# osudrl/cassie-mujoco-sim

Hardware: AMD Instinct MI355X
Metric: env-steps/sec (whole node) at N envs; max |qpos_err| vs CPU ref (higher is better)
Workload: dtype f64

## Files before the change

cassie-mujoco-sim_amd/cassie_amd/_lib.py:

```python
import ctypes
import os

from . import cstruct

PKG_DIR = os.path.dirname(os.path.dirname(os.path.abspath(__file__)))
REPO_DIR = os.path.dirname(PKG_DIR)
LIB_PATH = os.environ.get("CASSIE_LIB") or os.path.join(PKG_DIR, "lib", "libcassiemujoco.so")
MODEL_DIR = os.path.join(REPO_DIR, "models")

_variant_hdr = LIB_PATH + ".cm_model.h"
with open(_variant_hdr if os.path.exists(_variant_hdr) else os.path.join(PKG_DIR, "csrc", "cm_model.h")) as _f:
    _hdr = _f.read()
MACROS = cstruct.parse_defines(_hdr)
_structs = cstruct.parse_structs(_hdr, MACROS)
CmModel = _structs["cm_model_t"]
CmDriveState = _structs["cm_drive_state_t"]
CmEnvParams = _structs["cm_envparams_t"]
CmEpisodeRules = _structs.get("cm_episode_rules_t")

_lib = None


def lib():
    global _lib
# ... 74 lines not shown
    L.phys_batch_download_drive_state.argtypes = [vp, vp, c.c_int, c.c_int]
    L.phys_batch_uses_applied.argtypes = [vp]
    L.phys_batch_drive_pass.argtypes = [vp, c.c_int, vp]
    L.phys_batch_mark.argtypes = [vp]
    L.phys_batch_debug_poison_lds.argtypes = [vp]
    L.phys_batch_set_balance.argtypes = [vp, c.c_int]
    L.phys_batch_set_fast_rows.argtypes = [vp, c.c_int]
    L.phys_batch_set_waves_per_env.argtypes = [vp, c.c_int]
    L.phys_batch_set_inplace.argtypes = [vp, c.c_int]
    L.phys_batch_debug_inplace_ranges.argtypes = [vp]
    L.phys_batch_debug_form_launches.argtypes = [vp, c.POINTER(c.c_longlong), c.POINTER(c.c_longlong)]
    L.phys_batch_download_cost.argtypes = [vp, vp]
    L.phys_batch_measured_shader_clock.argtypes = [vp, vp]
    L.phys_batch_wide_pass_envs.argtypes = [vp, c.c_int]
    L.phys_batch_set_chunks.argtypes = [vp, c.c_int]
    L.phys_batch_debug_handover_pending.argtypes = [vp]
    L.phys_batch_debug_handover_pending.restype = c.c_int
    if hasattr(L, "phys_batch_kernel_timing"):
        L.phys_batch_enable_kernel_timing.argtypes = [vp, c.c_int]
        L.phys_batch_kernel_timing.argtypes = [vp, c.POINTER(c.c_int), c.POINTER(c.c_double)]
    if hasattr(L, "phys_batch_step_range"):
        L.phys_batch_step_range.argtypes = [vp, c.c_int, c.c_int, c.c_int, vp]
    if hasattr(L, "phys_batch_reset_envs"):
        L.phys_batch_reset_envs.argtypes = [vp, c.c_int, c.c_int, c.c_int, vp, vp, vp]
    if hasattr(L, "phys_batch_end_episodes"):
        L.phys_batch_episodes_enable.argtypes = [vp, c.POINTER(CmEpisodeRules)]
        L.phys_batch_episodes_set_bank.argtypes = [vp, vp, c.c_int, c.c_int]
        L.phys_batch_episode_row_dim.argtypes = [vp]
        L.phys_batch_episode_ptr.restype = vp
        L.phys_batch_episode_ptr.argtypes = [vp, c.c_int]
# ... 24 lines not shown
```

cassie-mujoco-sim_amd/cassie_amd/phys.py:

```python
import ctypes
import os

import numpy as np

from ._lib import CmDriveState, CmEnvParams, CmEpisodeRules, CmModel, MODEL_DIR, lib

(F_QPOS, F_QVEL, F_QACC_WARMSTART, F_TIME, F_CTRL, F_QFRC_APPLIED, F_XFRC_APPLIED, F_QACC, F_SENSORDATA,
 F_ACTUATOR_VELOCITY, F_XPOS, F_XQUAT, F_PD_PTARGET, F_PD_KP, F_PD_KD, F_BODY_CFRC, F_DRIVE_CMD, F_MEAS, F_PD_DTARGET,
 F_PD_TORQUE, F_DERIVED, F_QM, F_HEIGHT_SCAN) = range(23)

MAXV = 40
DRV_COM_POS, DRV_COM_VEL, DRV_ANGMOM, DRV_FOOT_POS, DRV_FOOT_VEL, DRV_FOOT_FORCE, DRV_TOE_FORCE, DRV_HEEL_FORCE, DRV_MASS = 0, 3, 6, 9, 15, 27, 39, 45, 51
DRV_FOOT_JACP, DRV_FOOT_JACR, DRV_DIM = 52, 52 + 6 * MAXV, 52 + 12 * MAXV

DRIVE_OFF, DRIVE_TORQUE, DRIVE_PD, DRIVE_PD_SAFE = 0, 1, 2, 3
SAFETY_MSG_LIMIT, SAFETY_MSG_TORQUE = 1, 2
MEAS_DRIVE_POS, MEAS_DRIVE_VEL, MEAS_DRIVE_TORQUE, MEAS_JOINT_POS, MEAS_JOINT_VEL = 0, 10, 20, 30, 36
MEAS_ORIENTATION, MEAS_ANGVEL, MEAS_LINACC, MEAS_MAG, MEAS_DIM = 42, 46, 49, 52, 56

FLAG_EULERDAMP, FLAG_WARMSTART, FLAG_REFSAFE, FLAG_HFDENSE, FLAG_HFMULTI, FLAG_HFPRISM, FLAG_BOX8 = 1, 2, 4, 8, 16, 32, 64
WARN_CONTACT_FULL, WARN_CONSTRAINT_FULL, WARN_UNSUPPORTED_PAIR, WARN_DIVERGED = 1, 2, 4, 8
WARN_CHUNK_PLACEMENT = 16
WARN_TERRAIN_INDEX = 32
WARN_SCAN_TILTED = 64
# ... 370 lines not shown
        a, c_ = ctypes.c_longlong(0), ctypes.c_longlong(0)
        lib().phys_batch_debug_form_launches(self._h, ctypes.byref(a), ctypes.byref(c_))
        return int(a.value), int(c_.value)

    def inplace_ranges(self):
        return lib().phys_batch_debug_inplace_ranges(self._h)

    def set_waves_per_env(self, waves=2):
        if lib().phys_batch_set_waves_per_env(self._h, int(waves)) != 0:
            raise ValueError("waves per env: 1 or 2")

    def set_chunks(self, chunks=4):
        if lib().phys_batch_set_chunks(self._h, int(chunks)) != 0:
            raise ValueError("chunks per env-launch: 1 .. 7")

    def launch_cost(self):
        out = np.zeros(self.nenv, dtype=np.uint32)
        if lib().phys_batch_download_cost(self._h, out.ctypes.data) != 0:
            raise RuntimeError("cost download failed (balancing is off or the batch is small)")
        return out.astype(np.float64) * 64.0

    def measured_shader_clock(self):
        import ctypes
        hz = ctypes.c_double(0.0)
        if lib().phys_batch_measured_shader_clock(self._h, ctypes.byref(hz)) != 0:
            return None
        return float(hz.value)

    def wide_pass_envs(self, env0=0):
        r = lib().phys_batch_wide_pass_envs(self._h, int(env0))
# ... 43 lines not shown
```

cassie-mujoco-sim_amd/csrc/env_step_rows.inc:

```
        int r_ = lane;
        int rtype = -1, rid = 0, rsub = 0;
        int nefc = 0, nefc_before_contacts = 0;
        double rpos = 0, rmargin = 0, rR = 1.0, rK = 0, rB = 0, rimp = 1.0;
        const bool need_imu = lastsub || io.all_outputs_every_substep || (io.drive_mode && sub + 2 == nsub);
        const bool need_pos = lastsub || io.drive_mode || io.all_outputs_every_substep;
        const bool issens = lane < m->nsensor && need_pos;
        const int ls = issens ? lane : 0;
        SensorConsts sens_c;
        double ycol[NVP];
        double jvel = 0, jws = 0;
        const bool lastcol = !WIDE && lane == NROW - 1;
        for (int pass = 0; pass < (WIDE ? 2 : 1); ++pass) {
        if constexpr (WIDE) {
            if (pass == 1 && nefc <= NROW) break;
            r_ = NROW * pass + lane; rtype = -1; rid = 0; rsub = 0; nefc = 0; jvel = 0; jws = 0;
            rpos = 0; rmargin = 0; rR = 1.0; rK = 0; rB = 0; rimp = 1.0;
        }
        {
            const int neq = m->neq;
            const bool eact = lane < neq && m->eq_active[lane < neq ? lane : 0] != 0;
            const unsigned long long eall = neq >= 64 ? ~0ull : (1ull << neq) - 1;
            if (wv::ballot(eact) == eall && 3 * neq <= capr) {
                if (r_ < 3 * neq) { rtype = CM_CNSTR_EQUALITY; rid = r_ / 3; rsub = r_ - 3 * rid; }
                nefc = 3 * neq;
// ... 206 lines not shown
            if (!WIDE && rtype == CM_CNSTR_EQUALITY && r_ < CM_MAXEQROW) {
                ex->eq_pos[r_] = rpos; ex->eq_id[r_] = rid;
#pragma unroll
                for (int k = 0; k < NVP; ++k) if (k < nv) ex->eq_J[r_][k] = ycol[k];
            }
            if (lane == 0) { int ne = 0; for (int e = 0; e < m->neq; ++e) if (m->eq_active[e] && ne + 3 <= capr) ne += 3; ex->ne = ne; }
            if (lane < ncon) {
                ex->con_geom1[lane] = m->geom_fullid[S.c_g1[lane]]; ex->con_geom2[lane] = m->geom_fullid[S.c_g2[lane]];
                ex->con_body1[lane] = m->geom_bodyid[S.c_g1[lane]]; ex->con_body2[lane] = m->geom_bodyid[S.c_g2[lane]];
                ex->con_dim[lane] = S.c_dim[lane]; ex->con_dist[lane] = S.c_dist[lane];
                for (int i = 0; i < 3; ++i) ex->con_pos[lane][i] = S.c_pos[lane][i];
                for (int i = 0; i < 9; ++i) ex->con_frame[lane][i] = S.c_frame[lane][i];
            }
        }
        int caddr = -1;
        const bool want_cfrc = io.body_cfrc && (sub == nsub - 1 || !io.integrate);
        if (io.ext || want_cfrc) {
            int acc = nefc_before_contacts;
            for (int c = 0; c < ncon; ++c) {
                const int dim = S.c_dim[c];
                if (dim != 1 && dim != 3) continue;
                const int nrow = dim == 1 ? 1 : 2 * (dim - 1);
                if (acc + nrow > capr) continue;
                if (c == lane) caddr = acc;
                acc += nrow;
            }
        }
        wv::sync();
        CK_STAMP(8);
```

cassie-mujoco-sim_amd/csrc/env_step_wave1.inc:

```
    if constexpr (NW == 2) {
        if (wid == 1) {
            for (int sub1 = sub_start;;) {
                const int pb = isbody ? b : 0;
                const double mass = P->body_mass[pb];
                double iner[3], imat[9];
                for (int i = 0; i < 3; ++i) iner[i] = P->body_inertia[pb][i];
                for (int i = 0; i < 9; ++i) imat[i] = m->body_imat[pb][i];
                CK_STAMP(35);
                wv::block_barrier();
                if (wv::opaque(S.cmd[0])) return -1;
                wv::set_priority<(FEAT & FEAT_HFIELD) != 0 ? CK_PRIO_W1_FJ_HFIELD : CK_PRIO_W1_FJ>();
                CK_STAMP(36);
                double ximat[9] = {1, 0, 0, 0, 1, 0, 0, 0, 1};
                if (isbody && b > 0) {
                    double xm[9];
                    for (int i = 0; i < 9; ++i) xm[i] = S.x.s.xmat[b][i];
                    for (int i = 0; i < 3; ++i)
                        for (int c = 0; c < 3; ++c) ximat[3 * i + c] = xm[3 * i] * imat[c] + xm[3 * i + 1] * imat[3 + c] + xm[3 * i + 2] * imat[6 + c];
                }
                double col[NVP], colh[NVP];
                mass_matrix_columns<NVP, TOPO, FEAT, NW>(io, S, m, env, ids, mass, iner, ximat, col, colh);
                wv::publish(&S.cmd[3], sub1 + 1);
                CK_STAMP(38);
                factor_pair_by_height<NVP, TOPO, 0>(m, P, h, S, col, colh, lane);
                constexpr bool park_colh = NVP > 32;
                if constexpr (park_colh) {
                    if (isdof) {
#pragma unroll
                        for (int i = 0; i < NVP; ++i) {
                            if (i >= TOPO::nv) continue;
                            if (i == k_) S.dinvH[k_] = colh[i];
                            else if (i > k_ && LP::col_has(i, k_)) S.LHp[LP::col_idx(i, k_)] = colh[i];
                        }
                    }
                    wv::sync();
                }
                wv::wait_for(&S.cmd[4], sub1 + 1);
                if (wv::opaque(S.cmd[0])) return -1;
                if (io.drive_mode) {
                    if (io.integrate) drive_level_io(io, S, m, env, lane, sub1 == nsub - 1);
                    wv::sync();
                }
                CK_STAMP(4);
                {
                    const int kd = isdof ? k_ : 0;
                    const double kdamp = P->dof_damping[kd], kstiff = PS->dof_stiffness[kd], kref = PS->dof_springref[kd];
                    const double kgear = m->dof_gear[kd], klo = m->dof_ctrl_lo[kd], khi = m->dof_ctrl_hi[kd];
                    const int kq = m->dof_qadr[kd], ka = m->dof_act[kd];
                    wv::wait_for(&S.cmd[1], sub1 + 1);
                    bias_forces_and_qfrc_smooth<NVP, (NVP > 32)>(io, S, m, env, ids, kdamp, kstiff, kref, kgear, klo, khi, kq, ka);
                }
                const bool lastsub1 = sub1 == nsub - 1 || !io.integrate;
                const bool need_imu1 = lastsub1 || io.all_outputs_every_substep || (io.drive_mode && sub1 + 2 == nsub);
                const bool issens1 = lane < m->nsensor && (lastsub1 || io.drive_mode || io.all_outputs_every_substep);
                const int ls1 = issens1 ? lane : 0;
                const SensorConsts sens_c1 = request_sensor_consts(m, ls1);
                const int aslot1 = sensors_before_solve(io, S, m, env, issens1, ls1, sens_c1, need_imu1, lastsub1);
                CK_STAMP(47);
                wv::block_barrier();
                wv::set_priority<CK_PRIO_W1_JP>();
                CK_STAMP(39);
                if constexpr (WIDE) {
                    int it1 = 0, ng1 = 0;
                    const double f1 = wide_solve<NVP, TOPO>(S, m, P, 1, wv::opaque(S.x.turn[0]), sub1, it1, ng1);
                    (&S.c_solimp[0][0])[NROW + lane] = f1;
                }
                if constexpr (park_colh) {
#pragma unroll
// ... 76 lines not shown
                    }
                    if (isdof) S.qacc[k_] = qacc;
                    const double av = pf_agear * S.qvel[pf_adof];
                    wv::sync();
                    CK_STAMP(12);
                    if (io.integrate) {
                        if constexpr (!stage_h_early) stage_factor_h<NVP, TOPO>(S, k_, isdof, nv, lcol, lrowh);
                        euler_step<NVP, TOPO>(S, m, lane, isdof, k_, nv, njnt, h, qacc, lcol, lrowh, dih, pf_kdamp, pf_ejt, pf_eqa, pf_eda);
                    }
                    CK_STAMP(13);
                    wv::block_barrier();
                    wv::set_priority<CK_PRIO_W1_EF>();
                    outputs_after_qacc(io, S, m, env, lane, isdof, k_, nu, qacc, aslot, sb, need_imu, lastsub, av, ncon, nefc, iters, nguarded);
                    CK_STAMP(14);
                }
                if (!io.integrate || ++sub1 >= nsub) return -1;
            }
        }
    }
```

cassie-mujoco-sim_amd/csrc/phys_batch.hip:

```cpp
#include <hip/hip_runtime.h>

#include <cstdio>
#include <cstdlib>
#include <cstring>
#include <string>
#include <utility>
#include <vector>

#include "cassie_phys.h"
#include "device_mem.h"
#include "small_kernels.h"
#include "step_launch.h"

void phys_set_last_error(const char *s);

constexpr int DEFAULT_CHUNKS_WHOLE = 7 , DEFAULT_CHUNKS_RANGE = 2, CHUNK_MIN_ENVS = 2048, CHUNK_MIN_SUBSTEPS = 5;
constexpr int DEFAULT_TRAY_WAVES = 2;

struct phys_batch {
    int nenv = 0, device = 0;
    cm_model_t host_model;
    DevBuf<cm_model_t> d_models;
    DevBuf<cm_envparams_t> d_envparams;
    int model_stride = 0;
    bool generic_kernel = false;
    int dim[PHYS_F_COUNT];
    int stride[PHYS_F_COUNT];
    DevBuf<double> d_field[PHYS_F_COUNT];
    DevBuf<int> d_warn, d_info;
    DevBuf<float> d_hfield;
    size_t hfield_stride = 0, hfield_floats = 0;
// ... 20 lines not shown
    std::vector<OrderSeg> order_segs;
    std::vector<int> order_ident;
    DevBuf<cm_ext_t> d_ext;
    bool timing = false;
    std::vector<std::pair<hipEvent_t, hipEvent_t>> ev_pool;
    size_t ev_used = 0;
    DevBuf<int> d_progress;
    int chunks = DEFAULT_CHUNKS_WHOLE, chunks_range = DEFAULT_CHUNKS_RANGE;
    bool chunks_default = true;
    DevBuf<int> d_chunk_flag;
    int chunk_seq = 0;
    bool chunks_allowed = true;
    std::vector<std::pair<hipStream_t, bool>> probed_streams;
    HostWords chunk_fault;
    bool chunk_fault_reported = false;
    DevBuf<int> d_handover_list, d_handover_count;
    HostWords handover_seen;
    DevBuf<int> d_handover_list2, d_handover_count2;
    HostWords handover_seen2;
    bool fast_rows = true;
    int inplace_mode = 2;
    struct RangeForm { int env0; bool inplace; };
    std::vector<RangeForm> range_forms;
    long long form_launches[2] = {0, 0};
    int waves_per_env = 2;
    int waves_per_env_tray = DEFAULT_TRAY_WAVES;
    DevBuf<double> d_scratch_out;
    bool episodes = false;
    cm_episode_rules_t ep_rules;
    DevBuf<char> d_ep[PHYS_EP_ARRAYS];
// ... 127 lines not shown
    launch_step<40, TopoCassieTray38, ck::FEAT_WAVEPAIRS, FAST_ROWS_TRAY>,
    launch_step<40, TopoCassieTray38, ck::FEAT_WAVEPAIRS, FAST_ROWS_TRAY, 2>,
    nullptr,
    launch_step<40, TopoCassieTray38, ck::FEAT_WAVEPAIRS, MID_ROWS, 1, true>,
    launch_step<40, TopoCassieTray38, ck::FEAT_WAVEPAIRS, MID_ROWS, 2, true>,
    nullptr,
};
static const ck::StepLauncher CASSIE_ALL_FORMS[ck::FORM_COUNT] = {launch_step<32, TopoCassie32, ck::FEAT_ALL>};
static const ck::StepLauncher TRAY_HFIELD_FORMS[ck::FORM_COUNT] = {launch_step<40, TopoCassieTray38, ck::FEAT_ALL>};
static const ck::StepLauncher GENERIC32_FORMS[ck::FORM_COUNT] = {launch_step<32, TopoRuntime, ck::FEAT_ALL>};
static const ck::StepLauncher GENERIC40_FORMS[ck::FORM_COUNT] = {launch_step<40, TopoRuntime, ck::FEAT_ALL>};

constexpr int SMALL_BATCH_NSUB = 4;
constexpr int SMALL_BATCH = 512;

static void set_chunks(phys_batch *b, ck::PhysIO &io, int n, int nsub, hipStream_t s) {
    io.nchunk = 1;
    if (!b->chunks_allowed || (n == b->nenv ? b->chunks : b->chunks_range) <= 1 || n < CHUNK_MIN_ENVS || n % 8 != 0 || nsub < 2 * CHUNK_MIN_SUBSTEPS ||
        !stream_may_chunk(b, s))
        return;
    const int range_chunks = b->chunks_default && nsub <= 25 ? 3 : b->chunks_range;
    const int most = nsub / CHUNK_MIN_SUBSTEPS, asked = n == b->nenv ? b->chunks : range_chunks;
    io.nchunk = asked < most ? asked : most;
    if (b->chunk_seq >= (1 << 24)) {
        (void)hipDeviceSynchronize();
        (void)hipMemsetAsync(b->d_chunk_flag, 0, sizeof(int) * (size_t)b->nenv, s);
        (void)hipStreamSynchronize(s);
        b->chunk_seq = 0;
    }
    io.chunk_seq = ++b->chunk_seq;
    io.chunk_flag = b->d_chunk_flag;
    io.chunk_fault = b->chunk_fault.dev();
}

static void range_lists(phys_batch *b, int env0, int n, bool wide, ck::HandoverLists &hl, ck::StepGrids &g) {
    hl.list1 = b->d_handover_list; hl.count1 = b->d_handover_count + 2 * (size_t)env0; hl.seen1 = b->handover_seen.dev() + env0;
    if (wide) { hl.list2 = b->d_handover_list2; hl.count2 = b->d_handover_count2 + 2 * (size_t)env0; hl.seen2 = b->handover_seen2.dev() + env0; }
    const int seen = b->handover_seen.host()[env0], seen2 = wide ? b->handover_seen2.host()[env0] : 0;
// ... 182 lines not shown
        if (f == PHYS_F_DERIVED || f == PHYS_F_QM) continue;
        if (f == PHYS_F_HEIGHT_SCAN) continue;
        ok = ok && b->d_field[f].alloc(n * (d[f] > 0 ? d[f] : 1), true, "field");
    }
    ok = ok && b->d_models.alloc(1, false, "model");
    ok = ok && hip_ok(hipMemcpy(b->d_models, model, sizeof(cm_model_t), hipMemcpyHostToDevice), "hipMemcpy(model)");
    ok = ok && b->d_warn.alloc(n, true, "warn") && b->d_info.alloc(4 * n, true, "info");
    if (nenv >= 2048) {
        b->order_ident.resize(n);
        for (int e = 0; e < nenv; ++e) b->order_ident[(size_t)e] = e;
        ok = ok && b->d_order.alloc(n, false, "order");
        ok = ok && hip_ok(hipMemcpy(b->d_order, b->order_ident.data(), sizeof(int) * n, hipMemcpyHostToDevice), "hipMemcpy(order)");
        ok = ok && b->d_cost.alloc(n, true, "cost") && b->d_cost_wall.alloc(n, true, "cost, wall clock");
    }
    ok = ok && b->d_progress.alloc(n, true, "progress") && b->d_chunk_flag.alloc(n, true, "chunk words");
    if (const char *ck = getenv("CASSIE_CHUNKS")) { b->chunks = b->chunks_range = atoi(ck) > 1 ? (atoi(ck) < 7 ? atoi(ck) : 7) : 1; b->chunks_default = false; }
    ok = ok && b->chunk_fault.alloc(1, "chunk fault word");
    ok = ok && b->d_handover_list.alloc(n, false, "hand-over list") && b->d_handover_count.alloc(2 * n, true, "hand-over counts");
    ok = ok && b->handover_seen.alloc(n, "hand-over seen");
    ok = ok && b->d_handover_list2.alloc(n, false, "second hand-over list") && b->d_handover_count2.alloc(2 * n, true, "second hand-over counts");
    ok = ok && b->handover_seen2.alloc(n, "second hand-over seen");
    ok = ok && hip_ok(hipStreamCreateWithFlags(&b->stream, hipStreamNonBlocking), "hipStreamCreate");
    ok = ok && hip_ok(hipEventCreate(&b->ev0), "hipEventCreate") && hip_ok(hipEventCreate(&b->ev1), "hipEventCreate");
    ok = ok && hip_ok(hipEventCreateWithFlags(&b->ev_mark, hipEventDisableTiming), "hipEventCreate");
    if (ok) {
        std::vector<double> q0((size_t)nenv * model->nq);
        for (int e = 0; e < nenv; ++e) memcpy(&q0[(size_t)e * model->nq], model->qpos0, sizeof(double) * model->nq);
        ok = hip_ok(hipMemcpy(b->d_field[PHYS_F_QPOS], q0.data(), q0.size() * sizeof(double), hipMemcpyHostToDevice),
                    "hipMemcpy(qpos0)");
    }
// ... 663 lines not shown
}

int phys_batch_set_inplace(phys_batch_t *b, int mode) {
    if (!b || mode < 0 || mode > 2) return -1;
    b->inplace_mode = mode;
    return 0;
}

int phys_batch_set_chunks(phys_batch_t *b, int chunks) {
    if (!b || chunks < 1 || chunks > 7) return -1;
    b->chunks = b->chunks_range = chunks;
    b->chunks_default = false;
    return 0;
}

int phys_batch_set_waves_per_env(phys_batch_t *b, int waves) {
    if (!b || (waves != 1 && waves != 2)) return -1;
    b->waves_per_env = waves;
    b->waves_per_env_tray = waves;
    return 0;
}

int phys_batch_download_cost(phys_batch_t *b, unsigned *host) {
    if (!b || !host || !b->d_cost) return -1;
    (void)hipSetDevice(b->device);
    return quiesce(b) && hip_ok(hipMemcpy(host, b->d_cost, sizeof(unsigned) * (size_t)b->nenv, hipMemcpyDeviceToHost), "cost download") ? 0 : -1;
}

int phys_batch_measured_shader_clock(phys_batch_t *b, double *hz) {
    if (!b || !hz || !b->d_cost || !b->d_cost_wall) return -1;
// ... 90 lines not shown
```

cassie-mujoco-sim_amd/csrc/physics_kernel.h:

```cpp
#ifndef CASSIE_PHYSICS_KERNEL_H
#define CASSIE_PHYSICS_KERNEL_H

#include <wave.h>

#include "cm_model.h"
#include "topo_static.h"

#include "pk_types.h"
#include "pk_math.h"
#include "pk_safety.h"
#include "pk_collision.h"
#include "pk_factor_solve.h"
#include "pk_stages.h"
#include "pk_wide_solve.h"

namespace ck {


constexpr int ENV_STEP_WENT_DOWN = 1 << 20;

template <int NVP, class TOPO, int FEAT, int MAXR, int NW>
WV_DEVICE int env_step(const PhysIO &io, EnvShared<NVP, LPack<TOPO, NVP>::count, MAXR> &S, int env, int sub_start, int nsub) {
    typedef LPack<TOPO, NVP> LP;
    static_assert(NW == 1 || NW == 2, "one or two wavefronts per env");
    static_assert(NW == 1 || TOPO::is_static, "the two-wave form exists for the compile-time topologies");
    const int wid = NW == 2 ? wv::wave_id() : 0;
    if constexpr (NW == 2) { if (wid == 0) wv::set_priority<CK_PRIO_W0>(); }
    constexpr int prio_kin = (FEAT & FEAT_HFIELD) != 0 ? CK_PRIO_W0 : CK_PRIO_W0_KIN;

    static_assert(LP::covers() && LP::distinct(), "packed factor rows must hold every ancestor pair, each in its own slot");
    typedef EnvShared<NVP, LPack<TOPO, NVP>::count, MAXR> SH_T;
    constexpr int MAXC = SH_T::MAXC;
    constexpr bool WIDE = SH_T::WIDE;
    static_assert(!WIDE || (NW == 2 && MAXR == WIDE_ROWS), "the 127-row instantiation spreads its solve over the two wavefronts of an env");
    const ModelPtr m_launch = (ModelPtr)(io.models + (size_t)env * io.model_stride);
    ModelPtr m = m_launch;
    const ParamPtr P = io.envparams ? (ParamPtr)(io.envparams + (size_t)env) : (ParamPtr)&m_launch->params;
// ... 51 lines not shown
    const LaneIds ids = {nbody, nv, broot, bend, kjnt, kbody, kjt, kda, kroot, kbend, kdesc};
    wv::sync();

#include "env_step_wave1.inc"

    const float *env_hfield = nullptr;
    if constexpr ((FEAT & FEAT_HFIELD) != 0) {
        bool clamped;
        env_hfield = terrain_grid(io.hfield, io.hfield_stride, io.hfield_index, io.hfield_nterrain, env, &clamped);
        if (clamped && lane == 0 && wid == 0) wv::atomic_or(io.warn + env, WARN_TERRAIN_INDEX);
    }

    bool bailed = false, bailed_down = false;
    int sub = sub_start;
    for (; sub < nsub; ++sub) {
        const bool lastsub = sub == nsub - 1 || !io.integrate;
        const bool need_quat = lastsub || io.ext != nullptr || io.all_outputs_every_substep || (io.drive_mode && sub + 2 == nsub);
        {
            bool badv = false;
            if (lane < nq) { double v = S.qpos[lane]; badv |= !(v == v) || fabs(v) > 1e10; }
            if (lane < nv) { double v = S.qvel[lane]; badv |= !(v == v) || fabs(v) > 1e10; }
            if (wv::ballot(badv) != 0ull) {
                warn |= WARN_DIVERGED;
                if constexpr (NW == 2) { if (lane == 0) S.cmd[0] = 1; wv::block_barrier(); }
                break;
            }
        }
        if (io.drive_mode) {
        } else if (io.pd_ptarget) {
            if (lane < nu) {
                const size_t o = (size_t)env * io.su + lane;
                const double ratio = m->act_gear[lane], tmax = m->act_ctrlrange[lane][1];
// ... 311 lines not shown
        } else bias_forces_and_qfrc_smooth<NVP>(io, S, m, env, ids, kdamp, kstiff, kref, kgear, klo, khi, kq, ka);
        const int pf_eq = lane < 3 * m->neq ? lane / 3 : 0;
        int pf_eb1 = m->eq_body1[pf_eq], pf_eb2 = m->eq_body2[pf_eq], pf_er1 = m->eq_root[pf_eq][0], pf_er2 = m->eq_root[pf_eq][1];

#include "env_step_rows.inc"

#include "env_step_solve.inc"

    if (io.progress && lane == 0 && (!io.resume || bailed)) {
        io.progress[env] = bailed ? sub : nsub;
        if (bailed && !bailed_down && io.handover_out_list) io.handover_out_list[io.env0 + wv::atomic_add(io.handover_out_count, 1)] = env;
    }
    if (io.integrate && io.drive_mode) {
        drive_state_store(io, S, env, lane);
        if (lane < nu) io.ctrl[(size_t)env * io.su + lane] = S.ctrl[lane];
        if (bailed) {
            if (lane < m->nsensordata) io.sensordata[(size_t)env * io.ssd + lane] = S.sens[lane];
            if (lane < nu) io.actuator_velocity[(size_t)env * io.su + lane] = S.actvel[lane];
            if (lane < CM_NUM_DRIVES) {
                double *meas = io.meas + (size_t)env * CM_MEAS_DIM;
                meas[CM_MEAS_DRIVE_POS + lane] = S.drv_pos[lane]; meas[CM_MEAS_DRIVE_VEL + lane] = S.drv_vel[lane];
            }
        }
    }
    if (io.integrate) {
        if (lane < nq) io.qpos[(size_t)env * io.sq + lane] = S.qpos[lane];
        if (lane < nv) {
            io.qvel[(size_t)env * io.sqv + lane] = S.qvel[lane];
            io.qacc_warmstart[(size_t)env * io.sv + lane] = S.qacc_ws[lane];
        }
        if (lane == 0) io.time[env] = time;
    }
    {
        int w = 0;
        for (int bit = 1; bit <= 8; bit <<= 1)
            if (wv::ballot((warn & bit) != 0) != 0ull) w |= bit;
        if (lane == 0 && w) io.warn[env] |= w;
    }
    return (warn & WARN_DIVERGED) ? -2 : (bailed ? (bailed_down ? sub | ENV_STEP_WENT_DOWN : sub) : nsub);
}

template <int NVP, class TOPO, int FEAT = FEAT_ALL, int MAXR = MID_ROWS, int NW = 1, bool WALK = false, int WPS = NW, int INROWS = 0>
WV_GLOBAL void __launch_bounds__(WV_WAVE * NW) WV_OCC WV_WAVES_PER_SIMD(WPS) cassie_step_kernel(PhysIO io) {
    WV_SHARED EnvShared<NVP, LPack<TOPO, NVP>::count, MAXR> S;
    const int slot = wv::env_id();
    if constexpr (WALK) {
        wv::test_launch_hook(&S, sizeof S);
        const int count = wv::opaque(wv::shfl_i(wv::lane() == 0 ? wv::atomic_add(io.handover_count, 0) : 0, 0));
        for (int idx = slot; idx < count; idx += wv::grid_size()) {
            const int env = io.handover_list[io.env0 + idx];
            const long long t0 = io.cost ? wv::clock() : 0, t0w = io.cost_wall ? wv::wall_clock() : 0;
            env_step<NVP, TOPO, FEAT, MAXR, NW>(io, S, env, io.progress[env], io.nsub);
            if (io.cost && wv::lane() == 0 && (NW == 1 || wv::wave_id() == 0)) {
                io.cost[env] += (unsigned)((wv::clock() - t0) >> 6);
                if (io.cost_wall) io.cost_wall[env] += (unsigned)(wv::wall_clock() - t0w);
            }
            if constexpr (NW == 2) wv::block_barrier();
            else wv::sync();
        }
        if (wv::lane() == 0 && (NW == 1 || wv::wave_id() == 0) && wv::atomic_add(io.handover_count + 1, 1) == wv::grid_size() - 1) {
            io.handover_count[0] = 0; io.handover_count[1] = 0;
            if (io.handover_seen) *io.handover_seen = count;
        }
    } else {
    const int chunk = io.nchunk > 1 ? wv::env_id() / io.nenv : 0;
    const int eslot = slot - chunk * io.nenv;
    if (chunk >= (io.nchunk > 1 ? io.nchunk : 1)) return;
    wv::test_launch_hook(&S, sizeof S);
    const int env = io.order ? io.order[io.env0 + eslot] : io.env0 + eslot;
    int sub_start = io.resume ? io.progress[env] : 0, sub_end = io.nsub;
    if (io.nchunk > 1) {
        const int per = (io.nsub + io.nchunk - 1) / io.nchunk;
        sub_start = chunk * per;
        sub_end = sub_start + per < io.nsub ? sub_start + per : io.nsub;
    }
    if (sub_start >= io.nsub) return;
    if (chunk > 0) {
        if (!wv::wait_global<NW>(io.chunk_flag + env, io.chunk_seq, chunk)) {
            if (wv::lane() == 0) { wv::atomic_or(io.warn + env, WARN_CHUNK_PLACEMENT); if (io.chunk_fault) *io.chunk_fault = 1; }
        }
        if (io.progress[env] != sub_start) {
            if (sub_end < io.nsub) wv::publish_global<NW>(io.chunk_flag + env, io.chunk_seq, chunk + 1);
            return;
        }
    }
    const long long t0 = io.cost ? wv::clock() : 0, t0w = io.cost_wall ? wv::wall_clock() : 0;
    if constexpr (INROWS > 0) {
        static_assert(NW == 2 && INROWS > MAXR && INROWS <= MID_ROWS, "the in-place form: a two-wave fast instantiation with the 63-row code behind it");
        static_assert(sizeof(EnvShared<NVP, LPack<TOPO, NVP>::count, MAXR>) == sizeof(EnvShared<NVP, LPack<TOPO, NVP>::count, INROWS>), "both instantiations use the env's LDS block alike");
        auto &S2 = reinterpret_cast<EnvShared<NVP, LPack<TOPO, NVP>::count, INROWS> &>(S);
        PhysIO io2 = io;
        io2.has_next = io.inplace_has_next; io2.handover_out_list = io.inplace_out_list; io2.handover_out_count = io.inplace_out_count;
        io2.down_rows = io.inplace_stay_rows;
        const bool stay = io.inplace_stay_rows > 0;
        bool did = false;
        for (int s = sub_start;;) {
            int at = env_step<NVP, TOPO, FEAT, MAXR, NW>(io, S, env, s, sub_end);
            if (wv::lane() == 0 && wv::wave_id() == 0) S.cmd[5] = at;
            wv::drain_vmem(); wv::block_barrier();
            at = wv::opaque(S.cmd[5]);
            if (at < 0 || at >= sub_end) break;
            did = true;
            int at2 = env_step<NVP, TOPO, FEAT, INROWS, NW>(io2, S2, env, at, stay ? sub_end : at + 1);
            if (wv::lane() == 0 && wv::wave_id() == 0) S.cmd[5] = at2;
            wv::drain_vmem(); wv::block_barrier();
            at2 = wv::opaque(S.cmd[5]);
            if (at2 < 0) break;
            const bool down = (at2 & ENV_STEP_WENT_DOWN) != 0;
            at2 &= ENV_STEP_WENT_DOWN - 1;
            if (at2 >= sub_end) break;
            if (stay ? !down : at2 != at + 1) break;
            s = at2;
        }
        if (did && io.inplace_count && wv::lane() == 0 && wv::wave_id() == 0) wv::atomic_add(io.inplace_count, 1);
    } else env_step<NVP, TOPO, FEAT, MAXR, NW>(io, S, env, sub_start, sub_end);
    if (sub_end < io.nsub) wv::publish_global<NW>(io.chunk_flag + env, io.chunk_seq, chunk + 1);
    if (io.prof && wv::lane() == 0) io.prof[(size_t)env * NSTAMP + 40 + (NW == 2 ? wv::wave_id() : 0)] = wv::hw_id();
    if (io.prof && wv::lane() == 0 && (NW == 1 || wv::wave_id() == 0)) {
        io.prof[(size_t)env * NSTAMP + 42] = wv::clock(); io.prof[(size_t)env * NSTAMP + 43] = wv::wall_clock();
    }
    if (io.cost && wv::lane() == 0 && (NW == 1 || wv::wave_id() == 0)) {
        const unsigned c = (unsigned)((wv::clock() - t0) >> 6);
        io.cost[env] = io.resume || chunk > 0 ? io.cost[env] + c : c;
        if (io.cost_wall) { const unsigned cw = (unsigned)(wv::wall_clock() - t0w); io.cost_wall[env] = io.resume || chunk > 0 ? io.cost_wall[env] + cw : cw; }
    }
    }
}

}
#endif
// ... 1 lines not shown
```

cassie-mujoco-sim_amd/csrc/pk_stages.h:

```cpp
#ifndef CASSIE_PK_STAGES_H
#define CASSIE_PK_STAGES_H

namespace ck {

WV_DEVICE int drive_sensor_slot(int i) { return i < 5 ? i : i + 3; }
WV_DEVICE int joint_sensor_slot(int j) { return j < 3 ? j + 5 : j + 10; }

#define WV_DRIVE_FN WV_DEVICE
template <class SH>
WV_DEVICE void drive_state_load(const PhysIO &io, SH &S, int env, int lane) {
    const cm_drive_state_t *ds = io.drive_state + env;
    const double *meas = io.meas + (size_t)env * CM_MEAS_DIM;
    if (lane < CM_NUM_DRIVES) {
        for (int k = 0; k < CM_DRIVE_FILTER_NB; ++k) S.drv_x[lane][k] = ds->drive_x[lane][k];
        for (int k = 0; k < CM_TORQUE_DELAY_CYCLES; ++k) S.drv_delay[lane][k] = ds->torque_delay[lane][k];
        S.drv_pos[lane] = meas[CM_MEAS_DRIVE_POS + lane]; S.drv_vel[lane] = meas[CM_MEAS_DRIVE_VEL + lane];
        if (lane == 0) S.drv_msg[0] = ds->safety_msg;
    } else if (lane < CM_NUM_DRIVES + CM_NUM_JOINTS) {
        const int j = lane - CM_NUM_DRIVES;
        for (int k = 0; k < CM_JOINT_FILTER_NB; ++k) S.drv_jx[j][k] = ds->joint_x[j][k];
        for (int k = 0; k < CM_JOINT_FILTER_NA; ++k) S.drv_jy[j][k] = ds->joint_y[j][k];
    }
}
template <class SH>
WV_DEVICE void drive_state_store(const PhysIO &io, SH &S, int env, int lane) {
    cm_drive_state_t *ds = io.drive_state + env;
    if (lane < CM_NUM_DRIVES) {
        for (int k = 0; k < CM_DRIVE_FILTER_NB; ++k) ds->drive_x[lane][k] = S.drv_x[lane][k];
        for (int k = 0; k < CM_TORQUE_DELAY_CYCLES; ++k) ds->torque_delay[lane][k] = S.drv_delay[lane][k];
        if (lane == 0) ds->safety_msg = S.drv_msg[0];
    } else if (lane < CM_NUM_DRIVES + CM_NUM_JOINTS) {
        const int j = lane - CM_NUM_DRIVES;
        for (int k = 0; k < CM_JOINT_FILTER_NB; ++k) ds->joint_x[j][k] = S.drv_jx[j][k];
        for (int k = 0; k < CM_JOINT_FILTER_NA; ++k) ds->joint_y[j][k] = S.drv_jy[j][k];
    }
}

enum { DRVC_RATIO = 0, DRVC_TMAX, DRVC_WMAX, DRVC_COUNTS, DRVC_SCALE, DRVC_U_OR_PT, DRVC_STO_OR_DT, DRVC_FF, DRVC_KP, DRVC_KD };
template <class SH>
WV_DEVICE void drive_consts_load(const PhysIO &io, SH &S, ModelPtr m, int env, int lane) {
    const double TWO_PI = 2 * 3.14159265358979323846, PI = 3.14159265358979323846;
    const int nu = m->nu;
    if (lane < CM_NUM_DRIVES) {
        const int i = lane, bits = m->sensor_bits[drive_sensor_slot(i)];
        const double ratio = m->act_gear[i], counts = (double)(1 << bits);
        double *c = S.drv_c[i];
        c[DRVC_RATIO] = ratio; c[DRVC_TMAX] = m->act_ctrlrange[i][1];
        c[DRVC_WMAX] = wv::div_rn(wv::mul_rn(wv::mul_rn(m->act_maxrpm[i], 2.0), PI), 60.0);
        c[DRVC_COUNTS] = counts; c[DRVC_SCALE] = wv::div_rn(wv::div_rn(TWO_PI, counts), ratio);
// ... 533 lines not shown
```

cassie-mujoco-sim_amd/csrc/pk_types.h:

```cpp
#ifndef CASSIE_PK_TYPES_H
#define CASSIE_PK_TYPES_H

namespace ck {

constexpr int NB = CM_MAXBODY;
constexpr int NG = CM_MAXGEOM;
constexpr int NROW = 64;
constexpr int MID_ROWS = CM_MAXEFC_NARROW;
constexpr int WIDE_ROWS = CM_MAXEFC;
constexpr int FAST_ROWS = 31;
constexpr int FAST_ROWS_TRAY = 47;
constexpr int NSTAMP = 48;
#define CK_TRI(k, i) ((k) * ((k) + 1) / 2 + (i))
#define CK_STAMP(i) do { if (io.prof && lane == 0) io.prof[(size_t)env * NSTAMP + (i)] = wv::clock(); CK_FRESH(); } while (0)
#define CK_FRESH() do { lane = wv::fresh_lane(); b = lane; k_ = lane; isbody = b < nbody; isdof = k_ < nv; } while (0)

enum { WARN_CONTACT_FULL = 1, WARN_CONSTRAINT_FULL = 2, WARN_UNSUPPORTED_PAIR = 4, WARN_DIVERGED = 8,
       WARN_CHUNK_PLACEMENT = 16 ,
       WARN_TERRAIN_INDEX = 32   ,
       WARN_SCAN_TILTED = 64      };

#ifndef WV_OCC
#define WV_OCC
#endif
// ... 35 lines not shown
    int resume;
    int nchunk, chunk_seq;
    int *chunk_flag;
    volatile int *chunk_fault;
    int *handover_list, *handover_count;
    volatile int *handover_seen;
    int has_next;
    int *handover_out_list, *handover_out_count;
    int inplace_has_next;
    int *inplace_out_list, *inplace_out_count;
    int inplace_stay_rows;
    int down_rows;
    int *inplace_count;
    const int *hfield_index;
    int hfield_nterrain;
};

WV_DEVICE const float *terrain_grid(const float *hfield, size_t stride, const int *index, int nterrain, int env, bool *clamped) {
    *clamped = false;
    if (!hfield) return nullptr;
    if (!index) return hfield + (size_t)env * stride;
    const int want = index[env], last = nterrain - 1;
    const int t = want > last ? last : (want < 0 ? 0 : want);
    *clamped = t != want;
    return hfield + (size_t)(t < 0 ? 0 : t) * stride;
}

template <int NVP>
struct BodyTiles {
    double xpos[NB][3], xquat[NB][4], xmat[NB][9], xipos[NB][3];
    double xanchor[CM_MAXJNT][3], xaxis[CM_MAXJNT][3];
// ... 52 lines not shown
```

include/cassie_phys.h:

```cpp
#ifndef CASSIE_PHYS_H
#define CASSIE_PHYS_H

#include <stddef.h>
#include "cm_model.h"

#ifdef __cplusplus
extern "C" {
#endif

typedef struct phys_model phys_model_t;

phys_model_t *phys_model_load(const char *path, char *err, int errlen);
phys_model_t *phys_model_copy(const phys_model_t *src);
void phys_model_free(phys_model_t *m);
int phys_model_save(const phys_model_t *m, const char *path);
void phys_model_set_const(phys_model_t *m);
int phys_model_compile(const phys_model_t *m, cm_model_t *out, char *err, int errlen);
unsigned phys_model_flags(const phys_model_t *m);
int phys_model_set_flag(phys_model_t *m, unsigned flag, int on);
unsigned long long phys_model_fingerprint(const phys_model_t *m);
unsigned long long phys_hash_floats(const float *data, size_t n);
int phys_model_name2id(const phys_model_t *m, int objtype, const char *name);
const char *phys_model_id2name(const phys_model_t *m, int objtype, int id);

// ... 95 lines not shown

int phys_batch_set_all_outputs_every_substep(phys_batch_t *b, int on);
int phys_batch_set_balance(phys_batch_t *b, int on);
int phys_batch_download_cost(phys_batch_t *b, unsigned *host);
int phys_batch_measured_shader_clock(phys_batch_t *b, double *hz);
int phys_batch_wide_pass_envs(phys_batch_t *b, int env0);
int phys_batch_debug_handover_pending(phys_batch_t *b);
int phys_batch_enable_kernel_timing(phys_batch_t *b, int on);
int phys_batch_kernel_timing(phys_batch_t *b, int *launches, double *total_ms);
int phys_batch_set_fast_rows(phys_batch_t *b, int on);
int phys_batch_set_inplace(phys_batch_t *b, int mode);
int phys_batch_debug_inplace_ranges(const phys_batch_t *b);
int phys_batch_debug_form_launches(const phys_batch_t *b, long long *plain, long long *inplace);
int phys_batch_set_waves_per_env(phys_batch_t *b, int waves);
int phys_batch_set_chunks(phys_batch_t *b, int chunks);
int phys_batch_download_progress(phys_batch_t *b, int *host);

int phys_batch_debug_poison_lds(phys_batch_t *b);

int phys_batch_set_generic_kernel(phys_batch_t *b, int on);

int phys_batch_profile_step(phys_batch_t *b, long long *host_stamps);
int phys_batch_profile_substeps(phys_batch_t *b, int nsub, long long *host_stamps);

size_t phys_sizeof_model(void);
const char *phys_last_error(void);

#ifdef __cplusplus
}
#endif
// ... 2 lines not shown
```

Before: 27.45 million.

## Add tapered and named chunk splits with hand-over-aware output gating

Substep chunks can now be uneven. A packed table of chunk ends is passed to the kernel, and sizes come either from a user-named split or from an optional taper that front-loads substeps for short range steps. Outputs that only the final substep needs (IMU, cfrc, drive inputs) are now keyed to the true last substep rather than the chunk end, so a chunk that is not last avoids that work when hand-over is on. Drive inputs are stored at chunk boundaries. Taper is off by default, so the default path mostly only changes when last-substep outputs are computed for each chunk.

```diff
diff --git a/cassie-mujoco-sim_amd/cassie_amd/_lib.py b/cassie-mujoco-sim_amd/cassie_amd/_lib.py
--- a/cassie-mujoco-sim_amd/cassie_amd/_lib.py
+++ b/cassie-mujoco-sim_amd/cassie_amd/_lib.py
@@ -112,6 +112,11 @@
     L.phys_batch_measured_shader_clock.argtypes = [vp, vp]
     L.phys_batch_wide_pass_envs.argtypes = [vp, c.c_int]
     L.phys_batch_set_chunks.argtypes = [vp, c.c_int]
+    if hasattr(L, "phys_batch_set_chunk_split"):
+        L.phys_batch_set_chunk_handover.argtypes = [vp, c.c_int]
+        L.phys_batch_set_chunk_taper.argtypes = [vp, c.c_int]
+        L.phys_batch_set_chunk_split.argtypes = [vp, vp, c.c_int]
+        L.phys_batch_chunks_in_effect.argtypes = [vp, vp]
     L.phys_batch_debug_handover_pending.argtypes = [vp]
     L.phys_batch_debug_handover_pending.restype = c.c_int
     if hasattr(L, "phys_batch_kernel_timing"):
diff --git a/cassie-mujoco-sim_amd/cassie_amd/phys.py b/cassie-mujoco-sim_amd/cassie_amd/phys.py
--- a/cassie-mujoco-sim_amd/cassie_amd/phys.py
+++ b/cassie-mujoco-sim_amd/cassie_amd/phys.py
@@ -408,6 +408,22 @@
         if lib().phys_batch_set_chunks(self._h, int(chunks)) != 0:
             raise ValueError("chunks per env-launch: 1 .. 7")
 
+    def set_chunk_handover(self, on=True):
+        lib().phys_batch_set_chunk_handover(self._h, 1 if on else 0)
+
+    def set_chunk_taper(self, on=True):
+        lib().phys_batch_set_chunk_taper(self._h, 1 if on else 0)
+
+    def set_chunk_split(self, sizes=()):
+        arr = np.asarray(list(sizes), dtype=np.int32)
+        if lib().phys_batch_set_chunk_split(self._h, arr.ctypes.data if len(arr) else None, len(arr)) != 0:
+            raise ValueError("a split is 2 .. 8 chunks of at least one substep, 255 substeps in all")
+
+    def chunks_in_effect(self):
+        sizes = np.zeros(8, dtype=np.int32)
+        k = lib().phys_batch_chunks_in_effect(self._h, sizes.ctypes.data)
+        return [int(v) for v in sizes[:k]]
+
     def launch_cost(self):
         out = np.zeros(self.nenv, dtype=np.uint32)
         if lib().phys_batch_download_cost(self._h, out.ctypes.data) != 0:
diff --git a/cassie-mujoco-sim_amd/csrc/env_step_rows.inc b/cassie-mujoco-sim_amd/csrc/env_step_rows.inc
--- a/cassie-mujoco-sim_amd/csrc/env_step_rows.inc
+++ b/cassie-mujoco-sim_amd/csrc/env_step_rows.inc
@@ -2,7 +2,7 @@
         int rtype = -1, rid = 0, rsub = 0;
         int nefc = 0, nefc_before_contacts = 0;
         double rpos = 0, rmargin = 0, rR = 1.0, rK = 0, rB = 0, rimp = 1.0;
-        const bool need_imu = lastsub || io.all_outputs_every_substep || (io.drive_mode && sub + 2 == nsub);
+        const bool need_imu = lastsub || io.all_outputs_every_substep || (io.drive_mode && sub + 2 == nlast);
         const bool need_pos = lastsub || io.drive_mode || io.all_outputs_every_substep;
         const bool issens = lane < m->nsensor && need_pos;
         const int ls = issens ? lane : 0;
@@ -244,7 +244,7 @@
             }
         }
         int caddr = -1;
-        const bool want_cfrc = io.body_cfrc && (sub == nsub - 1 || !io.integrate);
+        const bool want_cfrc = io.body_cfrc && (sub == nlast - 1 || !io.integrate);
         if (io.ext || want_cfrc) {
             int acc = nefc_before_contacts;
             for (int c = 0; c < ncon; ++c) {
diff --git a/cassie-mujoco-sim_amd/csrc/env_step_wave1.inc b/cassie-mujoco-sim_amd/csrc/env_step_wave1.inc
--- a/cassie-mujoco-sim_amd/csrc/env_step_wave1.inc
+++ b/cassie-mujoco-sim_amd/csrc/env_step_wave1.inc
@@ -38,7 +38,7 @@
                 wv::wait_for(&S.cmd[4], sub1 + 1);
                 if (wv::opaque(S.cmd[0])) return -1;
                 if (io.drive_mode) {
-                    if (io.integrate) drive_level_io(io, S, m, env, lane, sub1 == nsub - 1);
+                    if (io.integrate) drive_level_io(io, S, m, env, lane, sub1 == nlast - 1);
                     wv::sync();
                 }
                 CK_STAMP(4);
@@ -50,8 +50,8 @@
                     wv::wait_for(&S.cmd[1], sub1 + 1);
                     bias_forces_and_qfrc_smooth<NVP, (NVP > 32)>(io, S, m, env, ids, kdamp, kstiff, kref, kgear, klo, khi, kq, ka);
                 }
-                const bool lastsub1 = sub1 == nsub - 1 || !io.integrate;
-                const bool need_imu1 = lastsub1 || io.all_outputs_every_substep || (io.drive_mode && sub1 + 2 == nsub);
+                const bool lastsub1 = sub1 == nlast - 1 || !io.integrate;
+                const bool need_imu1 = lastsub1 || io.all_outputs_every_substep || (io.drive_mode && sub1 + 2 == nlast);
                 const bool issens1 = lane < m->nsensor && (lastsub1 || io.drive_mode || io.all_outputs_every_substep);
                 const int ls1 = issens1 ? lane : 0;
                 const SensorConsts sens_c1 = request_sensor_consts(m, ls1);
@@ -158,7 +158,11 @@
                     outputs_after_qacc(io, S, m, env, lane, isdof, k_, nu, qacc, aslot, sb, need_imu, lastsub, av, ncon, nefc, iters, nguarded);
                     CK_STAMP(14);
                 }
-                if (!io.integrate || ++sub1 >= nsub) return -1;
+                if (!io.integrate) return -1;
+                if (++sub1 >= nsub) {
+                    if (nsub < nlast) { wv::sync(); drive_inputs_store(io, S, m, env, lane, nu); }
+                    return -1;
+                }
             }
         }
     }
diff --git a/cassie-mujoco-sim_amd/csrc/phys_batch.hip b/cassie-mujoco-sim_amd/csrc/phys_batch.hip
--- a/cassie-mujoco-sim_amd/csrc/phys_batch.hip
+++ b/cassie-mujoco-sim_amd/csrc/phys_batch.hip
@@ -15,6 +15,7 @@
 void phys_set_last_error(const char *s);
 
 constexpr int DEFAULT_CHUNKS_WHOLE = 7 , DEFAULT_CHUNKS_RANGE = 2, CHUNK_MIN_ENVS = 2048, CHUNK_MIN_SUBSTEPS = 5;
+constexpr int TAPER_CHUNKS_SHORT = 4;
 constexpr int DEFAULT_TRAY_WAVES = 2;
 
 struct phys_batch {
@@ -65,6 +66,9 @@
     std::vector<std::pair<hipStream_t, bool>> probed_streams;
     HostWords chunk_fault;
     bool chunk_fault_reported = false;
+    bool chunk_handover = true, chunk_taper = false;
+    std::vector<int> chunk_split;
+    int chunks_last = 1, chunk_sizes_last[ck::CHUNK_TABLE] = {0};
     DevBuf<int> d_handover_list, d_handover_count;
     HostWords handover_seen;
     DevBuf<int> d_handover_list2, d_handover_count2;
@@ -222,14 +226,49 @@
 constexpr int SMALL_BATCH_NSUB = 4;
 constexpr int SMALL_BATCH = 512;
 
+static void taper_split(int nsub, int k, int *sizes) {
+    const int W = k * (k + 1) / 2;
+    int left = nsub;
+    for (int c = 0; c < k; ++c) { sizes[c] = nsub * (k - c) / W; left -= sizes[c]; }
+    for (int c = 0; left > 0; c = (c + 1) % k, --left) ++sizes[c];
+}
+constexpr int TAPER_MIN_LAST = 2;
+static int taper_chunks(int nsub, int asked) {
+    int k = 1;
+    while (k < asked && k < ck::CHUNK_TABLE && nsub / ((k + 1) * (k + 2) / 2) >= TAPER_MIN_LAST) ++k;
+    return k;
+}
+
 static void set_chunks(phys_batch *b, ck::PhysIO &io, int n, int nsub, hipStream_t s) {
-    io.nchunk = 1;
-    if (!b->chunks_allowed || (n == b->nenv ? b->chunks : b->chunks_range) <= 1 || n < CHUNK_MIN_ENVS || n % 8 != 0 || nsub < 2 * CHUNK_MIN_SUBSTEPS ||
+    io.nchunk = 1; io.chunk_ends = 0ull;
+    b->chunks_last = 1;
+    for (int c = 0; c < ck::CHUNK_TABLE; ++c) b->chunk_sizes_last[c] = c == 0 ? nsub : 0;
+    io.chunk_handover = b->chunk_handover ? 1 : 0;
+    int split_sum = 0;
+    for (int v : b->chunk_split) split_sum += v;
+    const bool named = b->chunk_split.size() > 1 && split_sum == nsub;
+    if (!b->chunks_allowed || (!named && ((n == b->nenv ? b->chunks : b->chunks_range) <= 1 || nsub < 2 * CHUNK_MIN_SUBSTEPS)) || n < CHUNK_MIN_ENVS || n % 8 != 0 ||
         !stream_may_chunk(b, s))
         return;
     const int range_chunks = b->chunks_default && nsub <= 25 ? 3 : b->chunks_range;
     const int most = nsub / CHUNK_MIN_SUBSTEPS, asked = n == b->nenv ? b->chunks : range_chunks;
     io.nchunk = asked < most ? asked : most;
+    int sizes[ck::CHUNK_TABLE] = {0};
+    if (named) {
+        io.nchunk = (int)b->chunk_split.size();
+        for (int c = 0; c < io.nchunk; ++c) sizes[c] = b->chunk_split[c];
+        io.chunk_ends = ck::chunk_ends_of(sizes, io.nchunk);
+    } else if (b->chunk_taper && b->chunk_handover && n != b->nenv && nsub <= 25) {
+        io.nchunk = taper_chunks(nsub, b->chunks_default ? TAPER_CHUNKS_SHORT : b->chunks_range);
+        taper_split(nsub, io.nchunk, sizes);
+        io.chunk_ends = ck::chunk_ends_of(sizes, io.nchunk);
+    } else {
+        const int per = (nsub + io.nchunk - 1) / io.nchunk;
+        for (int c = 0, at = 0; c < io.nchunk && c < ck::CHUNK_TABLE; ++c, at += per) sizes[c] = at + per < nsub ? per : (nsub > at ? nsub - at : 0);
+    }
+    b->chunks_last = io.nchunk;
+    for (int c = 0; c < ck::CHUNK_TABLE; ++c) b->chunk_sizes_last[c] = c < io.nchunk ? sizes[c] : 0;
+    if (io.nchunk <= 1) { io.nchunk = 1; io.chunk_ends = 0ull; return; }
     if (b->chunk_seq >= (1 << 24)) {
         (void)hipDeviceSynchronize();
         (void)hipMemsetAsync(b->d_chunk_flag, 0, sizeof(int) * (size_t)b->nenv, s);
@@ -442,6 +481,8 @@
         ok = ok && b->d_cost.alloc(n, true, "cost") && b->d_cost_wall.alloc(n, true, "cost, wall clock");
     }
     ok = ok && b->d_progress.alloc(n, true, "progress") && b->d_chunk_flag.alloc(n, true, "chunk words");
+    if (const char *ho = getenv("CASSIE_CHUNK_HANDOVER")) b->chunk_handover = atoi(ho) != 0;
+    if (const char *tp = getenv("CASSIE_CHUNK_TAPER")) b->chunk_taper = atoi(tp) != 0;
     if (const char *ck = getenv("CASSIE_CHUNKS")) { b->chunks = b->chunks_range = atoi(ck) > 1 ? (atoi(ck) < 7 ? atoi(ck) : 7) : 1; b->chunks_default = false; }
     ok = ok && b->chunk_fault.alloc(1, "chunk fault word");
     ok = ok && b->d_handover_list.alloc(n, false, "hand-over list") && b->d_handover_count.alloc(2 * n, true, "hand-over counts");
@@ -1135,6 +1176,31 @@
     return 0;
 }
 
+int phys_batch_set_chunk_handover(phys_batch_t *b, int on) {
+    if (!b) return -1;
+    b->chunk_handover = on != 0;
+    return 0;
+}
+
+int phys_batch_set_chunk_taper(phys_batch_t *b, int on) {
+    if (!b) return -1;
+    b->chunk_taper = on != 0;
+    return 0;
+}
+
+int phys_batch_set_chunk_split(phys_batch_t *b, const int *sizes, int n) {
+    if (!b || n < 0 || (n > 0 && !sizes)) return -1;
+    if (n > 0 && (n < 2 || ck::chunk_ends_of(sizes, n) == 0ull)) return -1;
+    b->chunk_split.assign(sizes, sizes + n);
+    return 0;
+}
+
+int phys_batch_chunks_in_effect(phys_batch_t *b, int *sizes) {
+    if (!b) return -1;
+    if (sizes) for (int c = 0; c < ck::CHUNK_TABLE; ++c) sizes[c] = b->chunk_sizes_last[c];
+    return b->chunks_last;
+}
+
 int phys_batch_set_waves_per_env(phys_batch_t *b, int waves) {
     if (!b || (waves != 1 && waves != 2)) return -1;
     b->waves_per_env = waves;
diff --git a/cassie-mujoco-sim_amd/csrc/physics_kernel.h b/cassie-mujoco-sim_amd/csrc/physics_kernel.h
--- a/cassie-mujoco-sim_amd/csrc/physics_kernel.h
+++ b/cassie-mujoco-sim_amd/csrc/physics_kernel.h
@@ -20,7 +20,7 @@
 constexpr int ENV_STEP_WENT_DOWN = 1 << 20;
 
 template <int NVP, class TOPO, int FEAT, int MAXR, int NW>
-WV_DEVICE int env_step(const PhysIO &io, EnvShared<NVP, LPack<TOPO, NVP>::count, MAXR> &S, int env, int sub_start, int nsub) {
+WV_DEVICE int env_step(const PhysIO &io, EnvShared<NVP, LPack<TOPO, NVP>::count, MAXR> &S, int env, int sub_start, int nsub, int nlast) {
     typedef LPack<TOPO, NVP> LP;
     static_assert(NW == 1 || NW == 2, "one or two wavefronts per env");
     static_assert(NW == 1 || TOPO::is_static, "the two-wave form exists for the compile-time topologies");
@@ -102,8 +102,8 @@
     bool bailed = false, bailed_down = false;
     int sub = sub_start;
     for (; sub < nsub; ++sub) {
-        const bool lastsub = sub == nsub - 1 || !io.integrate;
-        const bool need_quat = lastsub || io.ext != nullptr || io.all_outputs_every_substep || (io.drive_mode && sub + 2 == nsub);
+        const bool lastsub = sub == nlast - 1 || !io.integrate;
+        const bool need_quat = lastsub || io.ext != nullptr || io.all_outputs_every_substep || (io.drive_mode && sub + 2 == nlast);
         {
             bool badv = false;
             if (lane < nq) { double v = S.qpos[lane]; badv |= !(v == v) || fabs(v) > 1e10; }
@@ -445,14 +445,7 @@
     if (io.integrate && io.drive_mode) {
         drive_state_store(io, S, env, lane);
         if (lane < nu) io.ctrl[(size_t)env * io.su + lane] = S.ctrl[lane];
-        if (bailed) {
-            if (lane < m->nsensordata) io.sensordata[(size_t)env * io.ssd + lane] = S.sens[lane];
-            if (lane < nu) io.actuator_velocity[(size_t)env * io.su + lane] = S.actvel[lane];
-            if (lane < CM_NUM_DRIVES) {
-                double *meas = io.meas + (size_t)env * CM_MEAS_DIM;
-                meas[CM_MEAS_DRIVE_POS + lane] = S.drv_pos[lane]; meas[CM_MEAS_DRIVE_VEL + lane] = S.drv_vel[lane];
-            }
-        }
+        if (bailed || (NW == 1 && sub >= nsub && nsub < nlast)) drive_inputs_store(io, S, m, env, lane, nu);
     }
     if (io.integrate) {
         if (lane < nq) io.qpos[(size_t)env * io.sq + lane] = S.qpos[lane];
@@ -481,7 +474,7 @@
         for (int idx = slot; idx < count; idx += wv::grid_size()) {
             const int env = io.handover_list[io.env0 + idx];
             const long long t0 = io.cost ? wv::clock() : 0, t0w = io.cost_wall ? wv::wall_clock() : 0;
-            env_step<NVP, TOPO, FEAT, MAXR, NW>(io, S, env, io.progress[env], io.nsub);
+            env_step<NVP, TOPO, FEAT, MAXR, NW>(io, S, env, io.progress[env], io.nsub, io.nsub);
             if (io.cost && wv::lane() == 0 && (NW == 1 || wv::wave_id() == 0)) {
                 io.cost[env] += (unsigned)((wv::clock() - t0) >> 6);
                 if (io.cost_wall) io.cost_wall[env] += (unsigned)(wv::wall_clock() - t0w);
@@ -501,10 +494,17 @@
     const int env = io.order ? io.order[io.env0 + eslot] : io.env0 + eslot;
     int sub_start = io.resume ? io.progress[env] : 0, sub_end = io.nsub;
     if (io.nchunk > 1) {
-        const int per = (io.nsub + io.nchunk - 1) / io.nchunk;
-        sub_start = chunk * per;
-        sub_end = sub_start + per < io.nsub ? sub_start + per : io.nsub;
-    }
+        if (io.chunk_ends != 0ull) {
+            sub_start = chunk > 0 ? (int)((io.chunk_ends >> (8 * (chunk - 1))) & 255ull) : 0;
+            sub_end = (int)((io.chunk_ends >> (8 * chunk)) & 255ull);
+            if (sub_end > io.nsub) sub_end = io.nsub;
+        } else {
+            const int per = (io.nsub + io.nchunk - 1) / io.nchunk;
+            sub_start = chunk * per;
+            sub_end = sub_start + per < io.nsub ? sub_start + per : io.nsub;
+        }
+    }
+    const int out_end = io.chunk_handover ? io.nsub : sub_end;
     if (sub_start >= io.nsub) return;
     if (chunk > 0) {
         if (!wv::wait_global<NW>(io.chunk_flag + env, io.chunk_seq, chunk)) {
@@ -526,13 +526,14 @@
         const bool stay = io.inplace_stay_rows > 0;
         bool did = false;
         for (int s = sub_start;;) {
-            int at = env_step<NVP, TOPO, FEAT, MAXR, NW>(io, S, env, s, sub_end);
+            int at = env_step<NVP, TOPO, FEAT, MAXR, NW>(io, S, env, s, sub_end, out_end);
             if (wv::lane() == 0 && wv::wave_id() == 0) S.cmd[5] = at;
             wv::drain_vmem(); wv::block_barrier();
             at = wv::opaque(S.cmd[5]);
             if (at < 0 || at >= sub_end) break;
             did = true;
-            int at2 = env_step<NVP, TOPO, FEAT, INROWS, NW>(io2, S2, env, at, stay ? sub_end : at + 1);
+            const int end2 = stay ? sub_end : at + 1;
+            int at2 = env_step<NVP, TOPO, FEAT, INROWS, NW>(io2, S2, env, at, end2, io.chunk_handover ? io.nsub : end2);
             if (wv::lane() == 0 && wv::wave_id() == 0) S.cmd[5] = at2;
             wv::drain_vmem(); wv::block_barrier();
             at2 = wv::opaque(S.cmd[5]);
@@ -544,7 +545,7 @@
             s = at2;
         }
         if (did && io.inplace_count && wv::lane() == 0 && wv::wave_id() == 0) wv::atomic_add(io.inplace_count, 1);
-    } else env_step<NVP, TOPO, FEAT, MAXR, NW>(io, S, env, sub_start, sub_end);
+    } else env_step<NVP, TOPO, FEAT, MAXR, NW>(io, S, env, sub_start, sub_end, out_end);
     if (sub_end < io.nsub) wv::publish_global<NW>(io.chunk_flag + env, io.chunk_seq, chunk + 1);
     if (io.prof && wv::lane() == 0) io.prof[(size_t)env * NSTAMP + 40 + (NW == 2 ? wv::wave_id() : 0)] = wv::hw_id();
     if (io.prof && wv::lane() == 0 && (NW == 1 || wv::wave_id() == 0)) {
diff --git a/cassie-mujoco-sim_amd/csrc/pk_stages.h b/cassie-mujoco-sim_amd/csrc/pk_stages.h
--- a/cassie-mujoco-sim_amd/csrc/pk_stages.h
+++ b/cassie-mujoco-sim_amd/csrc/pk_stages.h
@@ -33,6 +33,16 @@
         const int j = lane - CM_NUM_DRIVES;
         for (int k = 0; k < CM_JOINT_FILTER_NB; ++k) ds->joint_x[j][k] = S.drv_jx[j][k];
         for (int k = 0; k < CM_JOINT_FILTER_NA; ++k) ds->joint_y[j][k] = S.drv_jy[j][k];
+    }
+}
+template <class SH>
+WV_DEVICE void drive_inputs_store(const PhysIO &io, SH &S, ModelPtr m, int env, int lane, int nu) {
+    if (!io.integrate || !io.drive_mode) return;
+    if (lane < m->nsensordata) io.sensordata[(size_t)env * io.ssd + lane] = S.sens[lane];
+    if (lane < nu) io.actuator_velocity[(size_t)env * io.su + lane] = S.actvel[lane];
+    if (lane < CM_NUM_DRIVES) {
+        double *meas = io.meas + (size_t)env * CM_MEAS_DIM;
+        meas[CM_MEAS_DRIVE_POS + lane] = S.drv_pos[lane]; meas[CM_MEAS_DRIVE_VEL + lane] = S.drv_vel[lane];
     }
 }
 
diff --git a/cassie-mujoco-sim_amd/csrc/pk_types.h b/cassie-mujoco-sim_amd/csrc/pk_types.h
--- a/cassie-mujoco-sim_amd/csrc/pk_types.h
+++ b/cassie-mujoco-sim_amd/csrc/pk_types.h
@@ -73,7 +73,22 @@
     int *inplace_count;
     const int *hfield_index;
     int hfield_nterrain;
+    int chunk_handover;
+    unsigned long long chunk_ends;
 };
+constexpr int CHUNK_TABLE = 8;
+inline unsigned long long chunk_ends_of(const int *sizes, int n) {
+    if (n < 1 || n > CHUNK_TABLE) return 0ull;
+    unsigned long long t = 0ull;
+    int end = 0;
+    for (int c = 0; c < n; ++c) {
+        if (sizes[c] < 1) return 0ull;
+        end += sizes[c];
+        if (end > 255) return 0ull;
+        t |= (unsigned long long)end << (8 * c);
+    }
+    return t;
+}
 
 WV_DEVICE const float *terrain_grid(const float *hfield, size_t stride, const int *index, int nterrain, int env, bool *clamped) {
     *clamped = false;
diff --git a/include/cassie_phys.h b/include/cassie_phys.h
--- a/include/cassie_phys.h
+++ b/include/cassie_phys.h
@@ -133,6 +133,10 @@
 int phys_batch_debug_form_launches(const phys_batch_t *b, long long *plain, long long *inplace);
 int phys_batch_set_waves_per_env(phys_batch_t *b, int waves);
 int phys_batch_set_chunks(phys_batch_t *b, int chunks);
+int phys_batch_set_chunk_handover(phys_batch_t *b, int on);
+int phys_batch_set_chunk_taper(phys_batch_t *b, int on);
+int phys_batch_set_chunk_split(phys_batch_t *b, const int *sizes, int n);
+int phys_batch_chunks_in_effect(phys_batch_t *b, int *sizes);
 int phys_batch_download_progress(phys_batch_t *b, int *host);
 
 int phys_batch_debug_poison_lds(phys_batch_t *b);
```

Result: no change. 27.22 million (-0.8%).
